# jameshensman/pyvb

Measured on AMD Instinct MI355X. Metric: VB update iterations/sec (T=10k, D=64, N=1024 LDS); ELBO rel-err vs NumPy, higher is better.
Workload: dtype f64; 1 GPU; LDS T=10000 D=64 K=64, 1024 replicates per GPU (BASELINE configs[2]); replicates_total=1024, parallelism=replicates sharded over 1 GPU(s), collective=none (1 GPU), degraded=False

## Files before the change

pyvb_amd/csrc/k_cols.hip:

```cpp
#include "params.h"

#define MFMA(a, b, c) __builtin_amdgcn_mfma_f64_16x16x4f64((a), (b), (c), 0, 0, 0)
#define MS 72
#define GS 68

__device__ __forceinline__ void load_row16(const double* row, int col0, int D, bool vec, double fill, double* out) {
    if (vec) {
#pragma unroll
        for (int g = 0; g < 4; ++g) {
            if (col0 + 4 * g < D) {
                const d4 v = *reinterpret_cast<const d4*>(row + col0 + 4 * g);
                out[4 * g] = v[0]; out[4 * g + 1] = v[1]; out[4 * g + 2] = v[2]; out[4 * g + 3] = v[3];
            } else {
                out[4 * g] = out[4 * g + 1] = out[4 * g + 2] = out[4 * g + 3] = fill;
            }
        }
    } else {
#pragma unroll
        for (int u = 0; u < 16; ++u) {
            const int c = col0 + u;
            const double v = row[c < D ? c : D - 1];
            out[u] = c < D ? v : fill;
        }
    }
}

__global__ void __launch_bounds__(64) k_cols(ParamArgs a) {
    const int WHICH = a.which0 + blockIdx.y;
    __shared__ double Mb[64 * MS];
    __shared__ double Gb[16 * GS];
    __shared__ double Sb[16 * GS];
    const int n = blockIdx.x, lane = threadIdx.x, D = a.D, K = a.K, c = lane & 15, q = lane >> 4;
    if (!a.active[n]) return;
    const int rows = WHICH == 0 ? D : K;
    double* M = (WHICH == 0 ? a.A_mean : a.C_mean) + (size_t)n * rows * D;
    double* V = (WHICH == 0 ? a.A_var : a.C_var) + (size_t)n * D * rows;
    double* qld = (WHICH == 0 ? a.qld_A : a.qld_C) + (size_t)n * D;
    double* lnd = (WHICH == 0 ? a.lnd_A : a.lnd_C) + (size_t)n * D;
    const double* pm = WHICH == 0 ? a.pri.A_pm : a.pri.C_pm;
    const double* pp = WHICH == 0 ? a.pri.A_pp : a.pri.C_pp;
    const double* obs = WHICH == 0 ? a.pri.A_obs : a.pri.C_obs;
    const double* mo = a.mom + (size_t)n * mom_total(D, K);
    const double* G = mo + (WHICH == 0 ? MOM_GA(D, K) : MOM_GC(D, K));
    const double* H = mo + (WHICH == 0 ? MOM_HA(D, K) : MOM_HC(D, K));
    const bool live = lane < rows;
    const int lr = live ? lane : 0;
    const int lc = lane < D ? lane : D - 1;
    const bool vec = (D & 3) == 0;
    const int nb = (D + 15) >> 4;
    const double* Mrow = M + (size_t)lr * D;
    const double* Hrow = H + (size_t)lr * D;

    for (int b = 0; b < 4; ++b) {
        double m[16] = {};
        if (b < nb) load_row16(Mrow, 16 * b, D, vec, 0.0, m);
#pragma unroll
        for (int u = 0; u < 16; ++u) Mb[(16 * b + u) * MS + lane] = (b < nb && live) ? m[u] : 0.0;
    }
    const double lam = live ? (WHICH == 0 ? a.Q_a[(size_t)n * D + lane] / a.Q_b[(size_t)n * D + lane]
                                          : a.R_a[(size_t)n * K + lane] / a.R_b[(size_t)n * K + lane]) : 0.0;

    auto stage_G = [&](int b) {
        double g[16];
#pragma unroll
        for (int u = 0; u < 16; ++u) {
            const int i = 16 * b + u;
            g[u] = G[(size_t)(i < D ? i : D - 1) * D + lc];
        }
#pragma unroll
        for (int u = 0; u < 16; ++u) Gb[u * GS + lane] = (16 * b + u < D && lane < D) ? g[u] : 0.0;
    };
    auto product = [&]() {
        d4 acc[4];
#pragma unroll
        for (int rt = 0; rt < 4; ++rt) acc[rt] = d4{0.0, 0.0, 0.0, 0.0};
#pragma unroll 4
        for (int s = 0; s < 16; ++s) {
            const double bop = Gb[c * GS + 4 * s + q];
#pragma unroll
            for (int rt = 0; rt < 4; ++rt) acc[rt] = MFMA(Mb[(4 * s + q) * MS + 16 * rt + c], bop, acc[rt]);
        }
#pragma unroll
        for (int rt = 0; rt < 4; ++rt)
#pragma unroll
            for (int r = 0; r < 4; ++r) Sb[c * GS + 16 * rt + 4 * r + q] = acc[rt][r];
    };

    if (a.c0 < a.c1) {
        for (int b = a.c0 >> 4; b <= (a.c1 - 1) >> 4; ++b) {
            __syncthreads();
            stage_G(b);
            double p0[16], m0[16], hk[16], ob[16];
#pragma unroll
            for (int u = 0; u < 16; ++u) {
                const int i = 16 * b + u;
                p0[u] = pp[(size_t)(i < D ? i : D - 1) * rows + lr];
            }
            load_row16(pm + (size_t)lr * D, 16 * b, D, vec, 0.0, m0);
            load_row16(Hrow, 16 * b, D, vec, 0.0, hk);
            load_row16(obs + (size_t)lr * D, 16 * b, D, vec, 0.0, ob);
            __syncthreads();
            product();
            __syncthreads();
            double gd[16], var[16], base[16];
#pragma unroll
            for (int u = 0; u < 16; ++u) {
                gd[u] = Gb[u * GS + 16 * b + u];
                const double prec = p0[u] + lam * gd[u];
                var[u] = 1.0 / prec;
                base[u] = p0[u] * m0[u] + lam * hk[u];
                p0[u] = prec;
            }
            double dl[16];
            int mynk = 0;
#pragma unroll
            for (int u = 0; u < 16; ++u) {
                const int i = 16 * b + u;
                dl[u] = 0.0;
                if (i >= a.c0 && i < a.c1) {
                    const double xo = Mb[i * MS + lane];
                    double acc = Sb[u * GS + lane] - xo * gd[u];
#pragma unroll
                    for (int v = 0; v < u; ++v) acc += dl[v] * Gb[u * GS + 16 * b + v];
                    double val = (base[u] - lam * acc) * var[u], vr = var[u];
                    const bool known = live && (ob[u] == ob[u]);
                    if (known) { val = ob[u]; vr = 0.0; }
                    const int nknown = __popcll(__ballot(known));
                    mynk = (lane == u) ? nknown : mynk;
                    if (live) {
                        dl[u] = val - xo;
                        Mb[i * MS + lane] = val;
                        V[(size_t)i * rows + lane] = vr;
                    }
                    Sb[u * GS + lane] = live ? p0[u] : 1.0;
                } else {
                    Sb[u * GS + lane] = 1.0;
                    mynk = (lane == u) ? rows : mynk;
                }
            }
            __syncthreads();
            {
                double mant = 1.0; int ex = 0;
#pragma unroll
                for (int r = 0; r < 16; ++r) {
                    int e;
                    mant *= frexp(Sb[c * GS + 16 * q + r], &e);
                    ex += e;
                }
#pragma unroll
                for (int o = 16; o <= 32; o <<= 1) {
                    mant *= __shfl_xor(mant, o, 64);
                    ex += __shfl_xor(ex, o, 64);
                }
                const int i = 16 * b + c;
                if (q == 0 && i >= a.c0 && i < a.c1 && mynk < rows) {
                    const double lp = log(mant) + (double)ex * 0.6931471805599453;
                    qld[i] = 0.5 / (0.5 * lp);
                    lnd[i] = -lp;
                }
            }
        }
        __syncthreads();
        if (live) {
            for (int b = a.c0 >> 4; b <= (a.c1 - 1) >> 4; ++b) {
#pragma unroll
                for (int g = 0; g < 4; ++g) {
                    const int cc = 16 * b + 4 * g;
                    if (vec) {
                        if (cc < D) {
                            d4 v;
#pragma unroll
                            for (int r = 0; r < 4; ++r) v[r] = Mb[(cc + r) * MS + lane];
                            *reinterpret_cast<d4*>(M + (size_t)lane * D + cc) = v;
                        }
                    } else {
#pragma unroll
                        for (int r = 0; r < 4; ++r)
                            if (cc + r < D) M[(size_t)lane * D + cc + r] = Mb[(cc + r) * MS + lane];
                    }
                }
            }
        }
    }

    if (a.fuse & 1) {
        double e0 = 0.0, e1 = 0.0, hm0 = 0.0, hm1 = 0.0;
        for (int b = 0; b < nb; ++b) {
            __syncthreads();
            stage_G(b);
            double hk[16], vv[16];
            load_row16(Hrow, 16 * b, D, vec, 0.0, hk);
#pragma unroll
            for (int u = 0; u < 16; ++u) {
                const int i = 16 * b + u;
                vv[u] = V[(size_t)(i < D ? i : D - 1) * rows + lr];
            }
            __syncthreads();
            product();
            __syncthreads();
#pragma unroll
            for (int u = 0; u < 16; u += 2) {
                const int i = 16 * b + u;
                const double x0 = Mb[i * MS + lane], x1 = Mb[(i + 1) * MS + lane];
                e0 += x0 * Sb[u * GS + lane] + (i < D ? vv[u] * Gb[u * GS + i] : 0.0);
                e1 += x1 * Sb[(u + 1) * GS + lane] + (i + 1 < D ? vv[u + 1] * Gb[(u + 1) * GS + i + 1] : 0.0);
                hm0 += x0 * hk[u];
                hm1 += x1 * hk[u + 1];
            }
        }
        const double own = WHICH == 0 ? mo[MOM_DP(D, K) + lr] : a.Syy[(size_t)n * K + lr];
        double r = 0.5 * own + 0.5 * (e0 + e1) - (hm0 + hm1);
        if (live) (WHICH == 0 ? a.resQ : a.resR)[(size_t)n * rows + lane] = r;
        if (a.fuse & 2) {
            const double* b0 = WHICH == 0 ? a.pri.Q_b0 : a.pri.R_b0;
            double* qb = (WHICH == 0 ? a.Q_b : a.R_b) + (size_t)n * rows;
            r = live ? r : 0.0;
            if (a.noise == PYVB_NOISE_GAMMA) {
                r = wave_sum(r);
                if (live) qb[lane] = b0[0] + r;
            } else if (live) {
                qb[lane] = b0[lane] + r;
            }
        }
    }
}

int launch_cols(pyvb_lds* h, int which, int c0, int c1, int fuse) {
    if (h->big) return launch_cols_big(h, which, c0, c1, fuse);
    ParamArgs a = make_args(h);
    a.c0 = c0; a.c1 = c1; a.which0 = which == 1 ? 1 : 0; a.fuse = fuse;
    TimedLaunch tl(h, PYVB_K_PARAMS);
    hipLaunchKernelGGL(k_cols, dim3(h->N, which == 2 ? 2 : 1), dim3(64), 0, h->stream, a);
    HIPCHK(hipGetLastError());
    return PYVB_OK;
}

int launch_resid(pyvb_lds* h, int which) { return launch_cols(h, which, 0, 0, 1); }
```

Before: 87.32 VB iterations/s per 1024 replicates (whole job).

## Drop LDS mean buffer; stream MFMA A-operand from global with register prefetch

Removes the 64x72 double shared-memory copy of the mean matrix. MFMA A operands are now loaded straight from global/L2 with a software-pipelined prefetch (sched_barriers), and updated columns are written back to global in groups of four inside the sweep. This cuts LDS footprint to raise occupancy (waves_per_eu 2) and drops the bulk staging and writeback passes. In exchange it depends on global reads seeing earlier in-kernel writes within the block, adds uncoalesced strided global loads, and raises register pressure.

```diff
diff --git a/pyvb_amd/csrc/k_cols.hip b/pyvb_amd/csrc/k_cols.hip
--- a/pyvb_amd/csrc/k_cols.hip
+++ b/pyvb_amd/csrc/k_cols.hip
@@ -1,7 +1,6 @@
 #include "params.h"
 
 #define MFMA(a, b, c) __builtin_amdgcn_mfma_f64_16x16x4f64((a), (b), (c), 0, 0, 0)
-#define MS 72
 #define GS 68
 
 __device__ __forceinline__ void load_row16(const double* row, int col0, int D, bool vec, double fill, double* out) {
@@ -25,9 +24,8 @@
     }
 }
 
-__global__ void __launch_bounds__(64) k_cols(ParamArgs a) {
+__global__ void __launch_bounds__(64) __attribute__((amdgpu_waves_per_eu(2))) k_cols(ParamArgs a) {
     const int WHICH = a.which0 + blockIdx.y;
-    __shared__ double Mb[64 * MS];
     __shared__ double Gb[16 * GS];
     __shared__ double Sb[16 * GS];
     const int n = blockIdx.x, lane = threadIdx.x, D = a.D, K = a.K, c = lane & 15, q = lane >> 4;
@@ -51,12 +49,9 @@
     const double* Mrow = M + (size_t)lr * D;
     const double* Hrow = H + (size_t)lr * D;
 
-    for (int b = 0; b < 4; ++b) {
-        double m[16] = {};
-        if (b < nb) load_row16(Mrow, 16 * b, D, vec, 0.0, m);
-#pragma unroll
-        for (int u = 0; u < 16; ++u) Mb[(16 * b + u) * MS + lane] = (b < nb && live) ? m[u] : 0.0;
-    }
+    const double* Ar[4];
+#pragma unroll
+    for (int rt = 0; rt < 4; ++rt) Ar[rt] = M + (size_t)min(16 * rt + c, rows - 1) * D;
     const double lam = live ? (WHICH == 0 ? a.Q_a[(size_t)n * D + lane] / a.Q_b[(size_t)n * D + lane]
                                           : a.R_a[(size_t)n * K + lane] / a.R_b[(size_t)n * K + lane]) : 0.0;
 
@@ -70,15 +65,37 @@
 #pragma unroll
         for (int u = 0; u < 16; ++u) Gb[u * GS + lane] = (16 * b + u < D && lane < D) ? g[u] : 0.0;
     };
+    auto load_A = [&](int g, double* out) {
+        int qq = q;
+        asm volatile("" : "+v"(qq));
+#pragma unroll
+        for (int s4 = 0; s4 < 4; ++s4) {
+            const int jc = min(16 * g + 4 * s4 + qq, D - 1);
+#pragma unroll
+            for (int rt = 0; rt < 4; ++rt) out[4 * s4 + rt] = Ar[rt][jc];
+        }
+    };
     auto product = [&]() {
         d4 acc[4];
 #pragma unroll
         for (int rt = 0; rt < 4; ++rt) acc[rt] = d4{0.0, 0.0, 0.0, 0.0};
-#pragma unroll 4
-        for (int s = 0; s < 16; ++s) {
-            const double bop = Gb[c * GS + 4 * s + q];
-#pragma unroll
-            for (int rt = 0; rt < 4; ++rt) acc[rt] = MFMA(Mb[(4 * s + q) * MS + 16 * rt + c], bop, acc[rt]);
+        double an[16];
+        __builtin_amdgcn_sched_barrier(0);
+        load_A(0, an);
+#pragma unroll
+        for (int g = 0; g < 4; ++g) {
+            double ac[16];
+#pragma unroll
+            for (int u = 0; u < 16; ++u) ac[u] = an[u];
+            __builtin_amdgcn_sched_barrier(0);
+            if (g < 3) load_A(g + 1, an);
+            __builtin_amdgcn_sched_barrier(0);
+#pragma unroll
+            for (int s4 = 0; s4 < 4; ++s4) {
+                const double bop = Gb[c * GS + 4 * (4 * g + s4) + q];
+#pragma unroll
+                for (int rt = 0; rt < 4; ++rt) acc[rt] = MFMA(ac[4 * s4 + rt], bop, acc[rt]);
+            }
         }
 #pragma unroll
         for (int rt = 0; rt < 4; ++rt)
@@ -90,25 +107,36 @@
         for (int b = a.c0 >> 4; b <= (a.c1 - 1) >> 4; ++b) {
             __syncthreads();
             stage_G(b);
-            double p0[16], m0[16], hk[16], ob[16];
+            double p0[16], base[16], xm[16];
+            unsigned kn = 0;
+            {
+                double m0[16], hk[16];
+#pragma unroll
+                for (int u = 0; u < 16; ++u) {
+                    const int i = 16 * b + u;
+                    p0[u] = pp[(size_t)(i < D ? i : D - 1) * rows + lr];
+                }
+                load_row16(pm + (size_t)lr * D, 16 * b, D, vec, 0.0, m0);
+                load_row16(Hrow, 16 * b, D, vec, 0.0, hk);
+#pragma unroll
+                for (int u = 0; u < 16; ++u) base[u] = p0[u] * m0[u] + lam * hk[u];
+            }
+            __syncthreads();
+            product();
+            load_row16(Mrow, 16 * b, D, vec, 0.0, xm);
+            {
+                double ob[16];
+                load_row16(obs + (size_t)lr * D, 16 * b, D, vec, 0.0, ob);
+#pragma unroll
+                for (int u = 0; u < 16; ++u)
+                    if (live && ob[u] == ob[u]) { base[u] = ob[u]; kn |= 1u << u; }
+            }
+            __syncthreads();
+            double var[16];
 #pragma unroll
             for (int u = 0; u < 16; ++u) {
-                const int i = 16 * b + u;
-                p0[u] = pp[(size_t)(i < D ? i : D - 1) * rows + lr];
-            }
-            load_row16(pm + (size_t)lr * D, 16 * b, D, vec, 0.0, m0);
-            load_row16(Hrow, 16 * b, D, vec, 0.0, hk);
-            load_row16(obs + (size_t)lr * D, 16 * b, D, vec, 0.0, ob);
-            __syncthreads();
-            product();
-            __syncthreads();
-            double gd[16], var[16], base[16];
-#pragma unroll
-            for (int u = 0; u < 16; ++u) {
-                gd[u] = Gb[u * GS + 16 * b + u];
-                const double prec = p0[u] + lam * gd[u];
+                const double prec = p0[u] + lam * Gb[u * GS + 16 * b + u];
                 var[u] = 1.0 / prec;
-                base[u] = p0[u] * m0[u] + lam * hk[u];
                 p0[u] = prec;
             }
             double dl[16];
@@ -118,18 +146,18 @@
                 const int i = 16 * b + u;
                 dl[u] = 0.0;
                 if (i >= a.c0 && i < a.c1) {
-                    const double xo = Mb[i * MS + lane];
-                    double acc = Sb[u * GS + lane] - xo * gd[u];
+                    const double xo = xm[u];
+                    double acc = Sb[u * GS + lane] - xo * Gb[u * GS + 16 * b + u];
 #pragma unroll
                     for (int v = 0; v < u; ++v) acc += dl[v] * Gb[u * GS + 16 * b + v];
                     double val = (base[u] - lam * acc) * var[u], vr = var[u];
-                    const bool known = live && (ob[u] == ob[u]);
-                    if (known) { val = ob[u]; vr = 0.0; }
+                    const bool known = (kn >> u) & 1;
+                    if (known) { val = base[u]; vr = 0.0; }
                     const int nknown = __popcll(__ballot(known));
                     mynk = (lane == u) ? nknown : mynk;
                     if (live) {
                         dl[u] = val - xo;
-                        Mb[i * MS + lane] = val;
+                        xm[u] = val;
                         V[(size_t)i * rows + lane] = vr;
                     }
                     Sb[u * GS + lane] = live ? p0[u] : 1.0;
@@ -137,6 +165,16 @@
                     Sb[u * GS + lane] = 1.0;
                     mynk = (lane == u) ? rows : mynk;
                 }
+                if ((u & 3) == 3 && live) {
+                    const int cc = 16 * b + u - 3;
+                    if (vec) {
+                        if (cc < D) *reinterpret_cast<d4*>(M + (size_t)lane * D + cc) = d4{xm[u - 3], xm[u - 2], xm[u - 1], xm[u]};
+                    } else {
+#pragma unroll
+                        for (int r = 0; r < 4; ++r)
+                            if (cc + r < D) M[(size_t)lane * D + cc + r] = xm[u - 3 + r];
+                    }
+                }
             }
             __syncthreads();
             {
@@ -160,27 +198,6 @@
                 }
             }
         }
-        __syncthreads();
-        if (live) {
-            for (int b = a.c0 >> 4; b <= (a.c1 - 1) >> 4; ++b) {
-#pragma unroll
-                for (int g = 0; g < 4; ++g) {
-                    const int cc = 16 * b + 4 * g;
-                    if (vec) {
-                        if (cc < D) {
-                            d4 v;
-#pragma unroll
-                            for (int r = 0; r < 4; ++r) v[r] = Mb[(cc + r) * MS + lane];
-                            *reinterpret_cast<d4*>(M + (size_t)lane * D + cc) = v;
-                        }
-                    } else {
-#pragma unroll
-                        for (int r = 0; r < 4; ++r)
-                            if (cc + r < D) M[(size_t)lane * D + cc + r] = Mb[(cc + r) * MS + lane];
-                    }
-                }
-            }
-        }
     }
 
     if (a.fuse & 1) {
@@ -188,8 +205,9 @@
         for (int b = 0; b < nb; ++b) {
             __syncthreads();
             stage_G(b);
-            double hk[16], vv[16];
+            double hk[16], vv[16], xm[16];
             load_row16(Hrow, 16 * b, D, vec, 0.0, hk);
+            load_row16(Mrow, 16 * b, D, vec, 0.0, xm);
 #pragma unroll
             for (int u = 0; u < 16; ++u) {
                 const int i = 16 * b + u;
@@ -201,7 +219,7 @@
 #pragma unroll
             for (int u = 0; u < 16; u += 2) {
                 const int i = 16 * b + u;
-                const double x0 = Mb[i * MS + lane], x1 = Mb[(i + 1) * MS + lane];
+                const double x0 = xm[u], x1 = xm[u + 1];
                 e0 += x0 * Sb[u * GS + lane] + (i < D ? vv[u] * Gb[u * GS + i] : 0.0);
                 e1 += x1 * Sb[(u + 1) * GS + lane] + (i + 1 < D ? vv[u + 1] * Gb[(u + 1) * GS + i + 1] : 0.0);
                 hm0 += x0 * hk[u];
```

After: 87.24 VB iterations/s per 1024 replicates (whole job). Within noise of the previous version (-0.1%).
